# ucuapps/OpenGlue

Measured on NVIDIA H100. Metric: image-pairs/sec at N=M=2048, d=256, 9 GNN layers, 100 Sinkhorn iters, higher is better.
Workload: dtype fp16x3 (fp16 hi/lo operands with power-of-two tensor scales, 3 products, fp32 accumulate)

## Files before the change

openglue_b200/csrc/api.cu:

```cuda
#include "common.cuh"
#include "linear_simt.cuh"
#include "linear_sm90.cuh"
#include "attention_simt.cuh"
#include "attention_sm90.cuh"
#include "sinkhorn.cuh"
#include "sinkhorn_bwd.cuh"
#include "match.cuh"
#include "gt_matches.cuh"
#include "criterion.cuh"
#include "metric_loss.cuh"
#include "collate.cuh"
#include "train_ops.cuh"
#include "superpoint.cuh"
#include "sift.cuh"
#include "kornia_sift.cuh"
#include "features.cuh"
#include "homography.cuh"
#include "optim.cuh"
#include <math.h>
#include <string.h>
#include <vector>

namespace og {

// ... 10 lines not shown
  float* o = out + (int64_t)r * (2 + S);
  if (len) {
    if (!padded_row_real(r, cap, len)) {
      for (int s = 0; s < 2 + S; ++s) o[s] = 0.f;
      return;
    }
    const int b = r / cap;
    wm1 = __ldg(wh + 4 * b) - 1.f;
    hm1 = __ldg(wh + 4 * b + 1) - 1.f;
  }
  o[0] = __fdiv_rn(2.f * __ldg(kpts + 2 * (int64_t)r), wm1) - 1.f;
  o[1] = __fdiv_rn(2.f * __ldg(kpts + 2 * (int64_t)r + 1), hm1) - 1.f;
  for (int s = 0; s < S; ++s) o[2 + s] = __ldg(side + (int64_t)r * S + s);
}

__global__ void __launch_bounds__(256) mask_padded_rows_kernel(const float* __restrict__ src, int64_t rows, int cap, int d,
                                                                const int* __restrict__ len, float* __restrict__ dst) {
  for (int64_t i = blockIdx.x * (int64_t)blockDim.x + threadIdx.x; i < rows * d; i += (int64_t)gridDim.x * blockDim.x)
    dst[i] = padded_row_real(i / d, cap, len) ? __ldg(src + i) : 0.f;
}

__global__ void __launch_bounds__(256) zero_padded_cols_kernel(float* __restrict__ ctx, int B, int d, int cap, const int* __restrict__ len) {
  for (int64_t i = blockIdx.x * (int64_t)blockDim.x + threadIdx.x; i < (int64_t)B * d * cap; i += (int64_t)gridDim.x * blockDim.x) {
    const int b = (int)(i / ((int64_t)d * cap));
    if ((int)(i % cap) >= padded_length(len, b, cap)) ctx[i] = 0.f;
  }
}

__global__ void sinkhorn_consts_kernel(SinkArgs a, float* out) {
  const int b = blockIdx.x * blockDim.x + threadIdx.x;
  if (b >= a.B) return;
  const SinkPair p(a, b);
  out[3 * b] = p.norm; out[3 * b + 1] = p.log_a_last; out[3 * b + 2] = p.log_b_last;
}

struct Layout {
  std::vector<int64_t> kenc_w, kenc_b;
  std::vector<int64_t> qkv_w, qkv_b, fc1_w, fc1_b, fc2_w, fc2_b;
  int64_t proj_w, proj_b, proj_rmix, dustbin, total;
  std::vector<int> kenc_sizes;
};

static int check_config(const og_config* c) {
  OG_CHECK_ARG(c != nullptr, "config is null");
  OG_CHECK_ARG(c->descriptor_dim > 0 && c->num_heads > 0 && c->descriptor_dim % c->num_heads == 0,
               "descriptor_dim %d must be a positive multiple of num_heads %d", c->descriptor_dim, c->num_heads);
  OG_CHECK_ARG(c->num_layers >= 0 && c->num_layers % 2 == 0, "num_layers must be 2 * num_stages");
  OG_CHECK_ARG(c->side_info_size >= 0, "side_info_size < 0");
  OG_CHECK_ARG(c->num_hidden >= 0 && c->num_hidden <= OG_MAX_HIDDEN, "num_hidden out of range");
  OG_CHECK_ARG(c->sinkhorn_iters >= 0 && c->sinkhorn_reg > 0.f, "bad sinkhorn parameters");
  OG_CHECK_ARG(c->descriptor_dim % 4 == 0, "descriptor_dim must be a multiple of 4");
  return OG_OK;
}

static Layout make_layout(const og_config* c) {
  Layout L;
  const int64_t d = c->descriptor_dim;
  L.kenc_sizes.push_back(2 + c->side_info_size);
  for (int i = 0; i < c->num_hidden; ++i) L.kenc_sizes.push_back(c->hidden[i]);
  L.kenc_sizes.push_back((int)d);
  int64_t off = 0;
  auto take = [&](int64_t nfl) { int64_t o = off; off += (nfl + 3) / 4 * 4; return o; };
  for (size_t i = 1; i < L.kenc_sizes.size(); ++i) {
    L.kenc_w.push_back(take((int64_t)L.kenc_sizes[i] * L.kenc_sizes[i - 1]));
    L.kenc_b.push_back(take(L.kenc_sizes[i]));
  }
  for (int l = 0; l < c->num_layers; ++l) {
    L.qkv_w.push_back(take(3 * d * d)); L.qkv_b.push_back(take(3 * d));
    L.fc1_w.push_back(take(4 * d * d)); L.fc1_b.push_back(take(2 * d));
    L.fc2_w.push_back(take(2 * d * d)); L.fc2_b.push_back(take(d));
  }
  L.proj_w = take(d * d); L.proj_b = take(d); L.proj_rmix = take(d); L.dustbin = take(1);
  L.total = off;
  return L;
}

struct Workspace {
  float *in0, *h0, *h1, *x, *qkv, *o, *hid, *g, *ghi, *glo, *sbuf;
  float *q, *khi, *klo, *vthi, *vtlo;
  int64_t ldn, ldm;
  void *sink, *match;
  float* slots;
  int nslots;
  float* desc;
  int64_t lds, sink_bytes, match_bytes, total;
};

static int plan_workspace(const og_config* c, int B, int n, int m, void* base, Workspace* w, bool padded = false) {
  const int64_t d = c->descriptor_dim, R = (int64_t)B * (n + m);
  int maxh = (int)d;
  for (int i = 0; i < c->num_hidden; ++i) maxh = std::max(maxh, c->hidden[i]);
  char* p = static_cast<char*>(base);
  int64_t off = 0;
  auto take = [&](int64_t bytes) { int64_t o = off; off += align_up(bytes, 256); return p ? (void*)(p + o) : nullptr; };
  w->in0 = (float*)take(R * (2 + c->side_info_size) * 4);
  w->h0 = (float*)take(R * maxh * 4);
  w->h1 = (float*)take(R * maxh * 4);
  w->x = (float*)take(R * d * 4);
  w->qkv = (float*)take(R * 3 * d * 4);
  w->o = (float*)take(R * d * 4);
  w->hid = (float*)take(R * 2 * d * 4);
  w->g = (float*)take(R * d * 4);
  w->ghi = (float*)take((int64_t)B * m * d * 4);
  w->glo = (float*)take((int64_t)B * m * d * 4);
  w->ldn = align_up(n, 8); w->ldm = align_up(m, 8);
  w->nslots = 16 * c->num_layers + 16;
  w->slots = (float*)take((int64_t)w->nslots * 4);
  if (c->precision == OG_PREC_TF32X3 || c->precision == OG_PREC_FP16X3) {
    w->q = (float*)take(R * d * 4);
    w->khi = (float*)take(R * d * 4);
    w->klo = (float*)take(R * d * 4);
    w->vthi = (float*)take((int64_t)B * d * (w->ldn + w->ldm) * 4);
    w->vtlo = (float*)take((int64_t)B * d * (w->ldn + w->ldm) * 4);
  } else {
    w->q = w->khi = w->klo = w->vthi = w->vtlo = nullptr;
  }
  w->lds = align_up(m, 4);
  w->sbuf = (float*)take((int64_t)B * n * w->lds * 4);
  w->sink_bytes = sinkhorn_workspace_bytes(B, n, m);
  if (w->sink_bytes < 0) return OG_EUNSUPPORTED;
  w->sink = take(w->sink_bytes);
  w->match_bytes = match_workspace_bytes(B, n, m);
  w->match = take(w->match_bytes);
  w->desc = padded ? (float*)take(R * d * 4) : nullptr;
  w->total = off;
  return OG_OK;
}

static og_linear_args lin(const float* A, int64_t lda, int k, const float* W, const float* bias, int rows, int nout,
                          float* Y, int64_t ldy) {
  og_linear_args a;
  memset(&a, 0, sizeof(a));
  a.A = A; a.lda = lda; a.k1 = k; a.W = W; a.ldw = k; a.bias = bias; a.rows = rows; a.nout = nout; a.batch = 1;
  a.alpha = 1.f; a.Y = Y; a.ldy = ldy;
  return a;
}

template <class T> static T gemm_args(const og_linear_args& a) {
  T t;
  memset(&t, 0, sizeof(t));
  t.A = a.A; t.lda = a.lda; t.strideA = a.strideA; t.A2 = a.A2; t.lda2 = a.lda2; t.strideA2 = a.strideA2;
  t.k1 = a.k1; t.k2 = a.k2;
  t.b_rows_per_batch = a.strideW ? (int)(a.strideW / a.ldw) : 0;
  t.bias = a.bias; t.rows = a.rows; t.nout = a.nout; t.batch = a.batch; t.alpha = a.alpha; t.relu = a.relu;
  t.R = a.R; t.ldr = a.ldr; t.strideR = a.strideR;
  if constexpr (std::is_same<T, TcLinearArgs>::value) {
    t.Y = a.Y; t.ldy = a.ldy; t.strideY = a.strideY; t.Yt = a.Yt; t.ldyt = a.ldyt; t.strideYt = a.strideYt; t.rscale = a.rscale;
  } else {
    t.out[F16_Y] = {a.Y, nullptr, nullptr, a.ldy, a.strideY, nullptr}; t.kind0 = F16_Y; t.nkinds = 1; t.kind_cols = a.nout;
  }
  return t;
}

template <class T, class BT>
static bool gemm_tileable(const og_linear_args& a, const T& t, const BT* Bhi, const BT* Blo) {
  return (!a.strideW || a.strideW % a.ldw == 0) && linear_sm90_eligible(t, Bhi, Blo, a.ldw);
}

template <class T, class BT>
static int gemm_launch(const og_linear_args& a, const T& t, const BT* Bhi, const BT* Blo, cudaStream_t s) {
  const int64_t brows = a.strideW ? (int64_t)t.b_rows_per_batch * (a.batch - 1) + a.nout : a.nout;
  return linear_sm90_launch(t, Bhi, Blo, a.ldw, brows, s);
}

template <class T, class BT>
static int linear_sm90_run(const og_linear_args& a, const T& t, const BT* Bhi, const BT* Blo, const char* who, const char* why,
                           cudaStream_t s) {
  if (!gemm_tileable(a, t, Bhi, Blo))
    return fail(OG_EUNSUPPORTED, "%s: %s", who, a.strideW && a.strideW % a.ldw != 0 ? "strideW must be a multiple of ldw" : why);
  return gemm_launch(a, t, Bhi, Blo, s);
}

struct SplitOut { float *Yhi = nullptr, *Ylo = nullptr, *Ythi = nullptr, *Ytlo = nullptr; };

static TcLinearArgs tc_args(const og_linear_args& a, const SplitOut& so) {
  TcLinearArgs t = gemm_args<TcLinearArgs>(a);
  t.Yhi = so.Yhi; t.Ylo = so.Ylo; t.Ythi = so.Ythi; t.Ytlo = so.Ytlo;
  return t;
}

static int linear_dispatch(const og_linear_args& a, int precision, cudaStream_t s, const float* Whi = nullptr,
                           const float* Wlo = nullptr, const SplitOut& so = SplitOut()) {
  if (precision == OG_PREC_TF32X3 && Whi && Wlo) {
    const TcLinearArgs t = tc_args(a, so);
    if (gemm_tileable(a, t, Whi, Wlo)) return gemm_launch(a, t, Whi, Wlo, s);
  }
  if (so.Yhi || so.Ythi) return fail(OG_EUNSUPPORTED, "split outputs need the tensor-core path");
// ... 935 lines not shown
                   overflow);
}
int og_mask_empty_pairs(const int* len0, const int* len1, int B, int n, int m, int64_t* matches0, float* mscores0, int64_t* matches1,
                        float* mscores1, void* stream) {
  OG_CHECK_ARG(len0 && len1 && matches0 && mscores0 && matches1 && mscores1, "mask_empty_pairs: null pointer");
  OG_CHECK_ARG(B > 0 && n > 0 && m > 0, "mask_empty_pairs: bad sizes");
  const int64_t total = (int64_t)B * ((int64_t)n + m);
  return OG_LAUNCH(mask_empty_pairs_kernel, eltwise_grid(total), 256, 0, (cudaStream_t)stream, len0, len1, B, n, m, matches0, mscores0,
                   matches1, mscores1);
}

int og_homography_pairs(const uint8_t* rgb, int B, int H, int W, int offset, const int32_t* warp_offset, float* image0, float* image1,
                        float* H_true, void* stream) {
  OG_CHECK_ARG(rgb && warp_offset && image0 && image1 && H_true, "homography_pairs: null pointer");
  OG_CHECK_ARG(B >= 1 && B <= 65535, "homography_pairs: B = %d must be in [1, 65535]", B);
  OG_CHECK_ARG(offset >= 1 && H > 0 && W > 0 && 2 * (int64_t)offset < (H < W ? H : W),
               "homography_pairs: offset %d must be >= 1 with 2 offset < min(H, W) = min(%d, %d)", offset, H, W);
  OG_CHECK_ARG((int64_t)HG_ROWS * W <= INT32_MAX, "homography_pairs: W = %d too large", W);
  const int h = H - 2 * offset;
  return OG_LAUNCH(homography_pairs_kernel, dim3(cdiv(h, HG_ROWS), B), HG_THREADS, 0, (cudaStream_t)stream, rgb, H, W, offset,
                   hg_block_width(H, W), warp_offset, image0, image1, H_true);
}

int64_t og_optim_state_bytes(void) { return (int64_t)sizeof(og_optim_state); }
int64_t og_optim_workspace_bytes(int nseg) { return nseg > 0 ? optim_workspace_bytes(nseg) : -1; }

static bool unit_beta(double b) { return b >= 0.0 && b < 1.0; }

static int clip_adam_impl(const og_optim_segment* segments, int nseg, int64_t ntiles, double beta1, double beta2, double eps,
                          double max_norm, double lr_gamma, og_optim_state* state, void* workspace, int64_t workspace_bytes,
                          const int* skip, void* stream) {
  OG_CHECK_ARG(segments && state && workspace, "clip_adam_step: null pointer");
  OG_CHECK_ARG(nseg > 0 && ntiles > 0, "clip_adam_step: nseg = %d and ntiles = %lld must be positive", nseg, (long long)ntiles);
  OG_CHECK_ARG(max_norm > 0.0, "clip_adam_step: max_norm = %g must be positive", max_norm);
  OG_CHECK_ARG(unit_beta(beta1) && unit_beta(beta2), "clip_adam_step: betas (%g, %g) must lie in [0, 1)", beta1, beta2);
  OG_CHECK_ARG(eps >= 0.0, "clip_adam_step: eps = %g must be >= 0", eps);
  OG_CHECK_ARG(lr_gamma > 0.0, "clip_adam_step: lr_gamma = %g must be positive", lr_gamma);
  if (workspace_bytes < optim_workspace_bytes(nseg)) return fail(OG_EWORKSPACE, "clip_adam_step: workspace too small");
  const OptHyper h = {beta1, beta2, eps, max_norm, lr_gamma};
  return optim_step_launch(segments, nseg, ntiles, h, state, workspace, skip, (cudaStream_t)stream);
}

int og_clip_adam_step(const og_optim_segment* segments, int nseg, int64_t ntiles, double beta1, double beta2, double eps,
                      double max_norm, double lr_gamma, og_optim_state* state, void* workspace, int64_t workspace_bytes, void* stream) {
  return clip_adam_impl(segments, nseg, ntiles, beta1, beta2, eps, max_norm, lr_gamma, state, workspace, workspace_bytes, nullptr, stream);
}

int og_clip_adam_step_guarded(const og_optim_segment* segments, int nseg, int64_t ntiles, double beta1, double beta2, double eps,
                              double max_norm, double lr_gamma, og_optim_state* state, void* workspace, int64_t workspace_bytes,
                              const int* skip, void* stream) {
  return clip_adam_impl(segments, nseg, ntiles, beta1, beta2, eps, max_norm, lr_gamma, state, workspace, workspace_bytes, skip, stream);
}

int og_adam_schedule(int64_t nsteps, double lr, double lr_gamma, double beta1, double beta2, double* lr_out, float* step_size,
                     float* bc2_sqrt, void* stream) {
  OG_CHECK_ARG(lr_out && step_size && bc2_sqrt, "adam_schedule: null pointer");
  OG_CHECK_ARG(nsteps > 0 && nsteps < (1 << 24), "adam_schedule: nsteps = %lld must lie in [1, 2^24)", (long long)nsteps);
  OG_CHECK_ARG(unit_beta(beta1) && unit_beta(beta2) && lr_gamma > 0.0, "adam_schedule: bad hyper-parameters");
  cudaStream_t st = (cudaStream_t)stream;
  if (const int rc = OG_LAUNCH(adam_lr_chain_kernel, 1, 1, 0, st, nsteps, lr, lr_gamma, lr_out)) return rc;
  return OG_LAUNCH(adam_scalars_kernel, (unsigned)std::min<int64_t>((nsteps + 255) / 256, 4096), 256, 0, st, nsteps, (const double*)lr_out,
                   beta1, beta2, step_size, bc2_sqrt);
}

static int forward_impl(const og_config* cfg, const float* Wp, const float* Whi, const float* Wlo, const __half* W16h,
                        const __half* W16l, const float* meta16, int B, int n, int m,
                         const float* kpts0,
                         const float* kpts1, const float* side0, const float* side1, const float* desc0,
                         const float* desc1, const float* img_wh, float* ctx0, float* ctx1, float* scores,
                         int64_t* matches0, float* mscores0, int64_t* matches1, float* mscores1, void* workspace,
                         int64_t workspace_bytes, void* stream_, const int* lens = nullptr, const float* pair_wh = nullptr) {
  int rc = check_config(cfg);
  if (rc != OG_OK) return rc;
  const bool padded = lens != nullptr;
  OG_CHECK_ARG(Wp && kpts0 && kpts1 && desc0 && desc1 && (padded ? pair_wh != nullptr : img_wh != nullptr) && scores && workspace,
               "forward: null pointer");
  OG_CHECK_ARG(cfg->side_info_size == 0 || (side0 && side1), "forward: side info missing");
  OG_CHECK_ARG(B > 0 && n > 0 && m > 0, "forward: batch, n, m must be positive");
  OG_CHECK_ARG(cfg->precision == OG_PREC_FP32 || (Whi && Wlo), "forward: the tensor-core modes need packed_hi / packed_lo");
  OG_CHECK_ARG(cfg->precision != OG_PREC_FP16X3 || (W16h && W16l && meta16), "forward: OG_PREC_FP16X3 needs the fp16 weight split (og_pack_f16)");
  const bool tcp = (cfg->precision != OG_PREC_FP32) && cfg->descriptor_dim >= 32;
  const bool f16p = tcp && cfg->precision == OG_PREC_FP16X3 && cfg->descriptor_dim % 64 == 0 &&
                    cfg->descriptor_dim / cfg->num_heads == 64;
  auto WH = [&](int64_t off) { return tcp ? Whi + off : nullptr; };
  auto WL = [&](int64_t off) { return tcp ? Wlo + off : nullptr; };
  OG_CHECK_ARG((reinterpret_cast<uintptr_t>(workspace) & 255) == 0, "forward: workspace must be 256-byte aligned");
  cudaStream_t st = (cudaStream_t)stream_;
  const int prec = cfg->precision == OG_PREC_FP16X3 ? OG_PREC_TF32X3 : cfg->precision;
  const Layout L = make_layout(cfg);
  Workspace w;
  rc = plan_workspace(cfg, B, n, m, workspace, &w, padded);
  if (rc != OG_OK) return rc;
  if (workspace_bytes < w.total) return fail(OG_EWORKSPACE, "forward: workspace %lld < %lld bytes",
                                             (long long)workspace_bytes, (long long)w.total);
  launch_counter() = 0;
  const int d = cfg->descriptor_dim, H = cfg->num_heads, dh = d / H, S = cfg->side_info_size;
  const int R0 = B * n, R1 = B * m, R = R0 + R1;
  float* x0 = w.x; float* x1 = w.x + (int64_t)R0 * d;

  const float* dsc0 = desc0;
  const float* dsc1 = desc1;
  const float wm0 = padded ? 0.f : img_wh[0] - 1.f, hm0 = padded ? 0.f : img_wh[1] - 1.f;
  const float wm1 = padded ? 0.f : img_wh[2] - 1.f, hm1 = padded ? 0.f : img_wh[3] - 1.f;
  const int* len0 = padded ? lens : nullptr;
  const int* len1 = padded ? lens + B : nullptr;
  const float* wh0 = padded ? pair_wh : nullptr;
  const float* wh1 = padded ? pair_wh + 2 : nullptr;
  if ((rc = OG_LAUNCH(kenc_input_kernel, cdiv(R0, 256), 256, 0, st, kpts0, side0, R0, S, wm0, hm0, n, len0, wh0, w.in0)) != OG_OK) return rc;
  if ((rc = OG_LAUNCH(kenc_input_kernel, cdiv(R1, 256), 256, 0, st, kpts1, side1, R1, S, wm1, hm1, m, len1, wh1,
                      w.in0 + (int64_t)R0 * (2 + S))) != OG_OK)
    return rc;
  if (padded) {
    float* d1m = w.desc + (int64_t)R0 * d;
    if ((rc = OG_LAUNCH(mask_padded_rows_kernel, eltwise_grid((int64_t)R0 * d), 256, 0, st, desc0, (int64_t)R0, n, d, lens, w.desc)) != OG_OK)
      return rc;
    if ((rc = OG_LAUNCH(mask_padded_rows_kernel, eltwise_grid((int64_t)R1 * d), 256, 0, st, desc1, (int64_t)R1, m, d, lens + B, d1m)) != OG_OK)
      return rc;
    dsc0 = w.desc; dsc1 = d1m;
  }
  {
    const float* cur = w.in0;
    float* bufs[2] = {w.h0, w.h1};
    const int nl = (int)L.kenc_sizes.size() - 1;
    for (int i = 0; i < nl; ++i) {
      const int kin = L.kenc_sizes[i], kout = L.kenc_sizes[i + 1];
      if (i < nl - 1) {
        og_linear_args a = lin(cur, kin, kin, Wp + L.kenc_w[i], Wp + L.kenc_b[i], R, kout, bufs[i & 1], kout);
        a.relu = 1;
        if ((rc = linear_dispatch(a, OG_PREC_FP32, st)) != OG_OK) return rc;
        cur = bufs[i & 1];
      } else {
        og_linear_args a = lin(cur, kin, kin, Wp + L.kenc_w[i], Wp + L.kenc_b[i], R0, kout, x0, d);
        if (!cfg->no_descriptors) { a.R = dsc0; a.ldr = d; }
        if ((rc = linear_dispatch(a, OG_PREC_FP32, st)) != OG_OK) return rc;
        og_linear_args b = lin(cur + (int64_t)R0 * kin, kin, kin, Wp + L.kenc_w[i], Wp + L.kenc_b[i], R1, kout, x1, d);
        if (!cfg->no_descriptors) { b.R = dsc1; b.ldr = d; }
        if ((rc = linear_dispatch(b, OG_PREC_FP32, st)) != OG_OK) return rc;
      }
    }
  }

  enum class Att { FP32, TF32, F16 };
  const Att att = f16p ? Att::F16 : (tcp && (dh == 32 || dh == 64)) ? Att::TF32 : Att::FP32;
  struct Seqs { int row0, len, count, img; int rows() const { return len * count; } };
  const Seqs img[2] = {{0, n, B, 0}, {R0, m, B, 1}};
  const Seqs all{0, R, 1, 2};
  const bool project_all_rows = att == Att::FP32, mlp_per_image = att == Att::F16;
  auto vt_ld = [&](const Seqs& kv) { return kv.row0 == 0 ? w.ldn : w.ldm; };
  auto vt_off = [&](const Seqs& kv) { return kv.row0 == 0 ? 0 : (int64_t)B * d * w.ldn; };

  int nslot = 0;
  auto new_slot = [&]() -> float* { return w.slots + (nslot < w.nslots - 1 ? nslot++ : w.nslots - 1); };
  float* sx[2] = {};
  struct SeqSlots { float *q, *k, *v, *o; } ss[2] = {};
  auto xslot = [&](const Seqs& g, int i) { return g.img == 2 ? sx[i] : i == 0 ? sx[g.img] : nullptr; };
  __half* kh16 = reinterpret_cast<__half*>(w.khi); __half* kl16 = reinterpret_cast<__half*>(w.klo);
  __half* vth16 = reinterpret_cast<__half*>(w.vthi); __half* vtl16 = reinterpret_cast<__half*>(w.vtlo);
  if (att == Att::F16) {
    OG_CUDA(cudaMemsetAsync(w.slots, 0, (size_t)w.nslots * 4, st));
    sx[0] = sx[1] = new_slot();
    const int64_t nx = (int64_t)R * d;
    if ((rc = OG_LAUNCH(amax_kernel, (unsigned)std::min<int64_t>((nx + 2047) / 2048, 1184), 256, 0, st, w.x, nx, sx[0])) != OG_OK) return rc;
  }
  auto args16 = [&](const og_linear_args& a, float* am0, float* am1, float* am2, int l, int t) {
    F16LinearArgs g = gemm_args<F16LinearArgs>(a);
    g.amax_in[0] = am0; g.amax_in[1] = am1; g.amax_in[2] = am2; g.w_meta = meta16 + ((int64_t)l * 5 + t) * 4;
// ... 50 lines not shown
    if (fuse_qkv && self) return run(q, F16_Y, 3);
    if (fuse_qkv) return (r = run(q, F16_Y, 1)) != OG_OK ? r : run(kv, F16_K, 2);
    for (int k = F16_Y; k < F16_KINDS; ++k)
      if ((r = run(k == F16_Y ? q : kv, k, 1)) != OG_OK) return r;
    return OG_OK;
  };

  auto attend = [&](const Seqs& q, const Seqs& kv) -> int {
    const float scale = (float)pow((double)dh, -0.5);
    const int* klen = padded ? lens + (kv.img == 1 ? B : 0) : nullptr;
    if (att == Att::FP32) {
      const float* qkv_q = w.qkv + (int64_t)q.row0 * 3 * d;
      const float* qkv_kv = w.qkv + (int64_t)kv.row0 * 3 * d;
      AttnArgs a{qkv_q, 3 * d, (int64_t)q.len * 3 * d, qkv_kv + d, 3 * d, (int64_t)kv.len * 3 * d, qkv_kv + 2 * d, 3 * d,
                 (int64_t)kv.len * 3 * d, w.o + (int64_t)q.row0 * d, d, (int64_t)q.len * d, q.count, q.len, kv.len, H, scale, klen};
      return attention_simt_launch(a, dh, st);
    }
    const int64_t ldv = vt_ld(kv), voff = vt_off(kv), k0 = (int64_t)kv.row0 * d;
    TcAttnArgs a{w.q + (int64_t)q.row0 * d, d, (int64_t)q.len * d, w.o + (int64_t)q.row0 * d, d, (int64_t)q.len * d,
                 q.count, q.len, kv.len, H, d, scale, klen};
    if (att == Att::TF32) return attention_tc_launch(a, w.khi + k0, w.klo + k0, d, w.vthi + voff, w.vtlo + voff, ldv, dh, st);
    const SeqSlots& s = ss[q.img == 1];
    return attention_f16_launch(a, F16AttnScales{s.q, s.k, s.v, s.o, 0}, kh16 + k0, kl16 + k0, d, vth16 + voff, vtl16 + voff, ldv, dh, st);
  };

  auto mlp = [&](int l, const Seqs& g) -> int {
    float* xr = w.x + (int64_t)g.row0 * d;
    float* hr = w.hid + (int64_t)g.row0 * 2 * d;
    og_linear_args a1 = lin(xr, d, d, Wp + L.fc1_w[l], Wp + L.fc1_b[l], g.rows(), 2 * d, hr, 2 * d);
    a1.A2 = w.o + (int64_t)g.row0 * d; a1.lda2 = d; a1.k2 = d; a1.ldw = 2 * d; a1.relu = 1;
    og_linear_args a2 = lin(hr, 2 * d, 2 * d, Wp + L.fc2_w[l], Wp + L.fc2_b[l], g.rows(), d, xr, d);
    a2.R = xr; a2.ldr = d;
    int r;
    if (att != Att::F16) {
      if ((r = linear_dispatch(a1, prec, st, WH(L.fc1_w[l]), WL(L.fc1_w[l]))) != OG_OK) return r;
      return linear_dispatch(a2, prec, st, WH(L.fc2_w[l]), WL(L.fc2_w[l]));
    }
    float* sh = new_slot();
    float* sn = new_slot();
    F16LinearArgs g1 = args16(a1, xslot(g, 0), xslot(g, 1), ss[g.img == 1].o, l, 3);
    g1.amax_out = sh;
    if ((r = run16(a1, g1, L.fc1_w[l])) != OG_OK) return r;
    F16LinearArgs g2 = args16(a2, sh, nullptr, nullptr, l, 4);
    g2.amax_out = sn;
    if ((r = run16(a2, g2, L.fc2_w[l])) != OG_OK) return r;
    if (g.img != 1) sx[0] = sn;
    if (g.img != 0) sx[1] = sn;
    return OG_OK;
  };

  for (int l = 0; l < cfg->num_layers; ++l) {
    if (l % 2 == 1) {
      for (int i = 0; i < 2; ++i) {
        if ((rc = project(l, img[i], img[1 - i])) != OG_OK) return rc;
        if ((rc = attend(img[i], img[1 - i])) != OG_OK) return rc;
        if ((rc = mlp(l, img[i])) != OG_OK) return rc;
      }
    } else if (n == m) {
      const Seqs both{0, n, 2 * B, 2};
      if ((rc = project(l, both, both)) != OG_OK) return rc;
      if ((rc = attend(both, both)) != OG_OK) return rc;
      if ((rc = mlp(l, both)) != OG_OK) return rc;
    } else {
      if (project_all_rows && (rc = project(l, all, all)) != OG_OK) return rc;
      for (int i = 0; i < 2; ++i) {
        if (!project_all_rows && (rc = project(l, img[i], img[i])) != OG_OK) return rc;
        if ((rc = attend(img[i], img[i])) != OG_OK) return rc;
      }
      for (int i = 0; i < (mlp_per_image ? 2 : 1); ++i)
        if ((rc = mlp(l, mlp_per_image ? img[i] : all)) != OG_OK) return rc;
    }
  }

  for (int img = 0; img < 2; ++img) {
    const int nn = img ? m : n;
    float* xr = img ? x1 : x0;
    float* gr = w.g + (img ? (int64_t)R0 * d : 0);
    og_linear_args a = lin(xr, d, d, Wp + L.proj_w, Wp + L.proj_b, nn, d, gr, d);
    a.batch = B; a.strideA = (int64_t)nn * d; a.strideY = (int64_t)nn * d;
    a.R = img ? dsc1 : dsc0; a.ldr = d; a.strideR = (int64_t)nn * d; a.rscale = Wp + L.proj_rmix;
    float* ctx = img ? ctx1 : ctx0;
    if (ctx) { a.Yt = ctx; a.ldyt = nn; a.strideYt = (int64_t)d * nn; }
    SplitOut so;
    if (tcp && img == 1) { so.Yhi = w.ghi; so.Ylo = w.glo; }
    if ((rc = linear_dispatch(a, prec, st, WH(L.proj_w), WL(L.proj_w), so)) != OG_OK) return rc;
    if (padded && ctx &&
        (rc = OG_LAUNCH(zero_padded_cols_kernel, eltwise_grid((int64_t)B * d * nn), 256, 0, st, ctx, B, d, nn, lens + (img ? B : 0))) != OG_OK)
      return rc;
  }
  {
    og_linear_args a = lin(w.g, d, d, w.g + (int64_t)R0 * d, nullptr, n, m, w.sbuf, w.lds);
    a.batch = B; a.strideA = (int64_t)n * d; a.strideW = (int64_t)m * d; a.strideY = (int64_t)n * w.lds;
    a.alpha = (float)pow((double)d, -0.5);
    if ((rc = linear_dispatch(a, prec, st, tcp ? w.ghi : nullptr, tcp ? w.glo : nullptr)) != OG_OK) return rc;
  }
  rc = sinkhorn_launch(w.sbuf, w.lds, (int64_t)n * w.lds, Wp + L.dustbin, B, n, m, cfg->sinkhorn_iters,
                       cfg->sinkhorn_reg, scores, w.sink, w.sink_bytes, st, nullptr, nullptr, lens);
  if (rc != OG_OK) return rc;
  if (matches0 || mscores0 || matches1 || mscores1) {
    rc = match_launch(scores, B, n, m, cfg->match_threshold, matches0, mscores0, matches1, mscores1, w.match,
                      w.match_bytes, st, lens);
    if (rc != OG_OK) return rc;
  }
  return OG_OK;
}

int og_superglue_forward(const og_config* cfg, const float* Wp, const float* Whi, const float* Wlo, int B, int n, int m,
                         const float* kpts0, const float* kpts1, const float* side0, const float* side1, const float* desc0,
                         const float* desc1, const float* img_wh, float* ctx0, float* ctx1, float* scores,
                         int64_t* matches0, float* mscores0, int64_t* matches1, float* mscores1, void* workspace,
                         int64_t workspace_bytes, void* stream) {
  if (cfg && cfg->precision == OG_PREC_FP16X3) return fail(OG_EINVAL, "forward: OG_PREC_FP16X3 takes og_superglue_forward_f16");
  return forward_impl(cfg, Wp, Whi, Wlo, nullptr, nullptr, nullptr, B, n, m, kpts0, kpts1, side0, side1, desc0, desc1, img_wh, ctx0, ctx1,
                      scores, matches0, mscores0, matches1, mscores1, workspace, workspace_bytes, stream);
}

int og_superglue_forward_f16(const og_config* cfg, const float* Wp, const float* Whi, const float* Wlo, const void* W16h,
                             const void* W16l, const float* meta16, int B, int n, int m,
                             const float* kpts0, const float* kpts1, const float* side0, const float* side1, const float* desc0,
                             const float* desc1, const float* img_wh, float* ctx0, float* ctx1, float* scores,
                             int64_t* matches0, float* mscores0, int64_t* matches1, float* mscores1, void* workspace,
                             int64_t workspace_bytes, void* stream) {
  return forward_impl(cfg, Wp, Whi, Wlo, static_cast<const __half*>(W16h), static_cast<const __half*>(W16l), meta16, B, n, m, kpts0, kpts1,
                      side0, side1, desc0, desc1, img_wh, ctx0, ctx1, scores, matches0, mscores0, matches1, mscores1, workspace,
                      workspace_bytes, stream);
}

int64_t og_workspace_bytes_padded(const og_config* cfg, int batch, int n, int m) {
  if (check_config(cfg) != OG_OK) return -1;
  if (batch <= 0 || n <= 0 || m <= 0) return fail(OG_EINVAL, "batch, n, m must be positive");
  Workspace w;
  if (plan_workspace(cfg, batch, n, m, nullptr, &w, true) != OG_OK) return -1;
  return w.total;
}

int og_superglue_forward_padded(const og_config* cfg, const float* Wp, const float* Whi, const float* Wlo, const void* W16h,
                                const void* W16l, const float* meta16, int B, int n, int m, const int* lengths,
                                const float* image_sizes, const float* kpts0, const float* kpts1, const float* side0,
                                const float* side1, const float* desc0, const float* desc1, float* ctx0, float* ctx1, float* scores,
                                int64_t* matches0, float* mscores0, int64_t* matches1, float* mscores1, void* workspace,
                                int64_t workspace_bytes, void* stream) {
  OG_CHECK_ARG(lengths && image_sizes, "forward_padded: null lengths / image_sizes");
  OG_CHECK_ARG(B <= 65535, "forward_padded: batch %d > 65535", B);
  return forward_impl(cfg, Wp, Whi, Wlo, static_cast<const __half*>(W16h), static_cast<const __half*>(W16l), meta16, B, n, m, kpts0, kpts1,
                      side0, side1, desc0, desc1, nullptr, ctx0, ctx1, scores, matches0, mscores0, matches1, mscores1, workspace,
                      workspace_bytes, stream, lengths, image_sizes);
}

int64_t og_f16_meta_floats(const og_config* cfg) {
  if (check_config(cfg) != OG_OK) return -1;
  return (int64_t)cfg->num_layers * 5 * 4;
}

int og_weight_split_f16(const float* w, const float* bias, int rows, int cols, void* hi16, void* lo16, float* meta, void* stream) {
  OG_CHECK_ARG(w && hi16 && lo16 && meta && rows > 0 && cols > 0, "weight_split_f16: bad arguments");
  cudaStream_t st = (cudaStream_t)stream;
  OG_CUDA(cudaMemsetAsync(meta, 0, 4 * sizeof(float), st));
  int rc;
  if ((rc = OG_LAUNCH(weight_meta_kernel, cdiv(rows, 8), 256, 0, st, w, bias, rows, cols, meta)) != OG_OK) return rc;
  const int64_t nel = (int64_t)rows * cols;
  if ((rc = OG_LAUNCH(split_f16_kernel, (unsigned)((nel + 255) / 256), 256, 0, st, w, static_cast<__half*>(hi16), static_cast<__half*>(lo16),
                      nel, meta)) != OG_OK)
    return rc;
  return OG_LAUNCH(finish_meta_kernel, 1, 1, 0, st, meta);
}

int og_pack_f16(const og_config* cfg, const float* Wp, void* hi16, void* lo16, float* meta, void* stream) {
  int rc = check_config(cfg);
  if (rc != OG_OK) return rc;
  OG_CHECK_ARG(Wp && hi16 && lo16 && meta, "pack_f16: null pointer");
  const Layout L = make_layout(cfg);
  const int64_t d = cfg->descriptor_dim;
  __half* h = static_cast<__half*>(hi16); __half* lo = static_cast<__half*>(lo16);
  for (int l = 0; l < cfg->num_layers; ++l) {
    struct T { int64_t woff, boff; int rows, cols; } ts[5] = {
      {L.qkv_w[l], L.qkv_b[l], (int)d, (int)d}, {L.qkv_w[l] + d * d, L.qkv_b[l] + d, (int)d, (int)d},
      {L.qkv_w[l] + 2 * d * d, L.qkv_b[l] + 2 * d, (int)d, (int)d},
      {L.fc1_w[l], L.fc1_b[l], (int)(2 * d), (int)(2 * d)}, {L.fc2_w[l], L.fc2_b[l], (int)d, (int)(2 * d)}};
    for (int t = 0; t < 5; ++t)
      if ((rc = og_weight_split_f16(Wp + ts[t].woff, Wp + ts[t].boff, ts[t].rows, ts[t].cols, h + ts[t].woff, lo + ts[t].woff,
                                    meta + ((int64_t)l * 5 + t) * 4, stream)) != OG_OK) return rc;
  }
  return OG_OK;
}
// ... 57 lines not shown
```

openglue_b200/csrc/match.cuh:

```cuda
#pragma once
#include "common.cuh"
#include <math_constants.h>

namespace og {

constexpr int MATCH_ROW_CHUNK = 64;

__device__ __forceinline__ int2 match_lengths(const int* lens, int b, int B, int n, int m) {
  if (!lens) return make_int2(n, m);
  return make_int2(padded_length(lens, b, n), padded_length(lens + B, b, m));
}

__global__ void __launch_bounds__(256) match_rowmax_kernel(const float* __restrict__ scores, int n, int m, const int* lens,
                                                            float* __restrict__ rowval, int* __restrict__ rowidx) {
  const int b = blockIdx.y;
  const int row = blockIdx.x * 8 + (threadIdx.x >> 5), lane = threadIdx.x & 31;
  const int2 len = match_lengths(lens, b, gridDim.y, n, m);
  if (row >= len.x) return;
  const float* src = scores + ((int64_t)b * (n + 1) + row) * (m + 1);
  float best = -CUDART_INF_F; int bi = 0x7fffffff;
  for (int c = lane; c < len.y; c += 32) {
    const float x = __ldg(src + c);
    if (x > best || bi == 0x7fffffff) { best = x; bi = c; }
  }
#pragma unroll
  for (int off = 16; off > 0; off >>= 1) {
    const float ov = __shfl_xor_sync(0xffffffffu, best, off);
    const int oi = __shfl_xor_sync(0xffffffffu, bi, off);
    if (ov > best || (ov == best && oi < bi)) { best = ov; bi = oi; }
  }
  if (lane == 0) { rowval[(int64_t)b * n + row] = best; rowidx[(int64_t)b * n + row] = bi; }
}

__global__ void __launch_bounds__(256) match_colmax_kernel(const float* __restrict__ scores, int n, int m, const int* lens, int chunks,
                                                            float* __restrict__ pval, int* __restrict__ pidx) {
  const int b = blockIdx.z, chunk = blockIdx.y;
  const int c = blockIdx.x * blockDim.x + threadIdx.x;
  const int2 len = match_lengths(lens, b, gridDim.z, n, m);
  if (c >= len.y) return;
  const int r0 = chunk * MATCH_ROW_CHUNK, r1 = min(r0 + MATCH_ROW_CHUNK, len.x);
  if (r0 >= r1) {
    pval[((int64_t)b * chunks + chunk) * m + c] = -CUDART_INF_F;
    pidx[((int64_t)b * chunks + chunk) * m + c] = r0;
    return;
  }
  const float* src = scores + (int64_t)b * (n + 1) * (m + 1) + c;
  float best = __ldg(src + (int64_t)r0 * (m + 1)); int bi = r0;
  for (int r = r0 + 1; r < r1; ++r) {
    const float x = __ldg(src + (int64_t)r * (m + 1));
    if (x > best) { best = x; bi = r; }
  }
  pval[((int64_t)b * chunks + chunk) * m + c] = best;
  pidx[((int64_t)b * chunks + chunk) * m + c] = bi;
}

__global__ void __launch_bounds__(256) match_colreduce_kernel(int n, int m, int chunks, const float* __restrict__ pval,
                                                               const int* __restrict__ pidx, int* __restrict__ colidx) {
  const int b = blockIdx.y;
  const int c = blockIdx.x * blockDim.x + threadIdx.x;
  if (c >= m) return;
  float best = pval[((int64_t)b * chunks) * m + c]; int bi = pidx[((int64_t)b * chunks) * m + c];
  for (int k = 1; k < chunks; ++k) {
    const float x = pval[((int64_t)b * chunks + k) * m + c];
    if (x > best) { best = x; bi = pidx[((int64_t)b * chunks + k) * m + c]; }
  }
  colidx[(int64_t)b * m + c] = bi;
}

__global__ void __launch_bounds__(256) match_finalize_kernel(int n, int m, const int* lens, float thr, const float* __restrict__ rowval,
                                                              const int* __restrict__ rowidx, const int* __restrict__ colidx,
                                                              int64_t* __restrict__ matches0, float* __restrict__ mscores0,
                                                              int64_t* __restrict__ matches1, float* __restrict__ mscores1) {
  const int b = blockIdx.y;
  const int t = blockIdx.x * blockDim.x + threadIdx.x;
  const int* ri = rowidx + (int64_t)b * n;
  const int* ci = colidx + (int64_t)b * m;
  const float* rv = rowval + (int64_t)b * n;
  const int2 len = match_lengths(lens, b, gridDim.y, n, m);
  if (t >= len.x && t < n) {
    if (matches0) matches0[(int64_t)b * n + t] = -1;
    if (mscores0) mscores0[(int64_t)b * n + t] = 0.f;
  }
  if (t >= len.y && t < m) {
    if (matches1) matches1[(int64_t)b * m + t] = -1;
    if (mscores1) mscores1[(int64_t)b * m + t] = 0.f;
  }
  if (t < len.x) {
    const int j = ri[t];
    const bool mutual = (ci[j] == t);
    const float ms = mutual ? expf(rv[t]) : 0.f;
    const bool valid = mutual && (ms > thr);
    if (matches0) matches0[(int64_t)b * n + t] = valid ? (int64_t)j : -1;
    if (mscores0) mscores0[(int64_t)b * n + t] = ms;
  }
  if (t < len.y && (matches1 || mscores1)) {
    const int i = ci[t];
    const bool mutual1 = (ri[i] == t);
    const bool mutual0_i = (ci[ri[i]] == i);
    const float ms0_i = mutual0_i ? expf(rv[i]) : 0.f;
    const float ms1 = mutual1 ? ms0_i : 0.f;
    const bool valid1 = mutual1 && (mutual0_i && ms0_i > thr);
    if (matches1) matches1[(int64_t)b * m + t] = valid1 ? (int64_t)i : -1;
    if (mscores1) mscores1[(int64_t)b * m + t] = ms1;
  }
}

inline int64_t match_workspace_bytes(int B, int n, int m) {
  const int chunks = cdiv(n, MATCH_ROW_CHUNK);
  return align_up((int64_t)B * n * 4, 256) * 2 + align_up((int64_t)B * m * 4, 256) +
         align_up((int64_t)B * chunks * m * 4, 256) * 2;
}

inline int match_launch(const float* scores, int B, int n, int m, float thr, int64_t* matches0, float* mscores0, int64_t* matches1,
                        float* mscores1, void* ws, int64_t ws_bytes, cudaStream_t stream, const int* lens = nullptr) {
  if (ws_bytes < match_workspace_bytes(B, n, m)) return fail(OG_EWORKSPACE, "match: workspace too small");
  const int chunks = cdiv(n, MATCH_ROW_CHUNK);
  char* w = static_cast<char*>(ws);
  float* rowval = reinterpret_cast<float*>(w); w += align_up((int64_t)B * n * 4, 256);
  int* rowidx = reinterpret_cast<int*>(w); w += align_up((int64_t)B * n * 4, 256);
  int* colidx = reinterpret_cast<int*>(w); w += align_up((int64_t)B * m * 4, 256);
  float* pval = reinterpret_cast<float*>(w); w += align_up((int64_t)B * chunks * m * 4, 256);
  int* pidx = reinterpret_cast<int*>(w);
  int rc;
  if ((rc = OG_LAUNCH(match_rowmax_kernel, dim3(cdiv(n, 8), B), 256, 0, stream, scores, n, m, lens, rowval, rowidx))) return rc;
  if ((rc = OG_LAUNCH(match_colmax_kernel, dim3(cdiv(m, 256), chunks, B), 256, 0, stream, scores, n, m, lens, chunks, pval, pidx)))
    return rc;
  if ((rc = OG_LAUNCH(match_colreduce_kernel, dim3(cdiv(m, 256), B), 256, 0, stream, n, m, chunks, pval, pidx, colidx))) return rc;
  return OG_LAUNCH(match_finalize_kernel, dim3(cdiv(std::max(n, m), 256), B), 256, 0, stream, n, m, lens, thr, rowval, rowidx,
                   colidx, matches0, mscores0, matches1, mscores1);
}

}
```

Before: 504.5.

## Run score GEMM in fp16x3 and fuse row/column argmax into one pass

For fp16x3 mode the descriptor score GEMM now runs on the fp16 sm90 GEMM. The second image's projected descriptors are split into fp16 hi/lo with amax-derived scales, instead of the tf32 hi/lo split. The match step also drops the separate row-max kernel: the column-max kernel now computes per-column-block row partial argmaxes via warp shuffles and shared memory, and finalize reduces those partials. This saves a full read of the score matrix and moves the score GEMM to cheaper fp16 tensor-core math, at the cost of extra amax/split launches and slightly different tie-breaking.

```diff
diff --git a/openglue_b200/csrc/api.cu b/openglue_b200/csrc/api.cu
--- a/openglue_b200/csrc/api.cu
+++ b/openglue_b200/csrc/api.cu
@@ -116,6 +116,7 @@
   void *sink, *match;
   float* slots;
   int nslots;
+  float* gmeta;
   float* desc;
   int64_t lds, sink_bytes, match_bytes, total;
 };
@@ -137,6 +138,7 @@
   w->g = (float*)take(R * d * 4);
   w->ghi = (float*)take((int64_t)B * m * d * 4);
   w->glo = (float*)take((int64_t)B * m * d * 4);
+  w->gmeta = (float*)take(8 * 4);
   w->ldn = align_up(n, 8); w->ldm = align_up(m, 8);
   w->nslots = 16 * c->num_layers + 16;
   w->slots = (float*)take((int64_t)w->nslots * 4);
@@ -1238,6 +1240,7 @@
   const bool tcp = (cfg->precision != OG_PREC_FP32) && cfg->descriptor_dim >= 32;
   const bool f16p = tcp && cfg->precision == OG_PREC_FP16X3 && cfg->descriptor_dim % 64 == 0 &&
                     cfg->descriptor_dim / cfg->num_heads == 64;
+  const bool f16_scores = tcp && cfg->precision == OG_PREC_FP16X3 && cfg->descriptor_dim % 64 == 0;
   auto WH = [&](int64_t off) { return tcp ? Whi + off : nullptr; };
   auto WL = [&](int64_t off) { return tcp ? Wlo + off : nullptr; };
   OG_CHECK_ARG((reinterpret_cast<uintptr_t>(workspace) & 255) == 0, "forward: workspace must be 256-byte aligned");
@@ -1454,7 +1457,7 @@
     float* ctx = img ? ctx1 : ctx0;
     if (ctx) { a.Yt = ctx; a.ldyt = nn; a.strideYt = (int64_t)d * nn; }
     SplitOut so;
-    if (tcp && img == 1) { so.Yhi = w.ghi; so.Ylo = w.glo; }
+    if (tcp && !f16_scores && img == 1) { so.Yhi = w.ghi; so.Ylo = w.glo; }
     if ((rc = linear_dispatch(a, prec, st, WH(L.proj_w), WL(L.proj_w), so)) != OG_OK) return rc;
     if (padded && ctx &&
         (rc = OG_LAUNCH(zero_padded_cols_kernel, eltwise_grid((int64_t)B * d * nn), 256, 0, st, ctx, B, d, nn, lens + (img ? B : 0))) != OG_OK)
@@ -1464,14 +1467,28 @@
     og_linear_args a = lin(w.g, d, d, w.g + (int64_t)R0 * d, nullptr, n, m, w.sbuf, w.lds);
     a.batch = B; a.strideA = (int64_t)n * d; a.strideW = (int64_t)m * d; a.strideY = (int64_t)n * w.lds;
     a.alpha = (float)pow((double)d, -0.5);
-    if ((rc = linear_dispatch(a, prec, st, tcp ? w.ghi : nullptr, tcp ? w.glo : nullptr)) != OG_OK) return rc;
+    if (f16_scores) {
+      __half* g1h = reinterpret_cast<__half*>(w.ghi); __half* g1l = reinterpret_cast<__half*>(w.glo);
+      float* am0 = w.gmeta + 4;
+      const int64_t n0 = (int64_t)R0 * d, n1 = (int64_t)R1 * d;
+      OG_CUDA(cudaMemsetAsync(w.gmeta, 0, 8 * sizeof(float), st));
+      if ((rc = OG_LAUNCH(amax_kernel, (unsigned)std::min<int64_t>((n1 + 2047) / 2048, 1184), 256, 0, st, a.W, n1, w.gmeta)) != OG_OK) return rc;
+      if ((rc = OG_LAUNCH(split_f16_kernel, (unsigned)((n1 + 255) / 256), 256, 0, st, a.W, g1h, g1l, n1, w.gmeta)) != OG_OK) return rc;
+      if ((rc = OG_LAUNCH(finish_meta_kernel, 1, 1, 0, st, w.gmeta)) != OG_OK) return rc;
+      if ((rc = OG_LAUNCH(amax_kernel, (unsigned)std::min<int64_t>((n0 + 2047) / 2048, 1184), 256, 0, st, w.g, n0, am0)) != OG_OK) return rc;
+      F16LinearArgs g = gemm_args<F16LinearArgs>(a);
+      g.amax_in[0] = am0; g.w_meta = w.gmeta;
+      if ((rc = linear_sm90_run(a, g, g1h, g1l, "forward", "the score GEMM is not tileable by the fp16 GEMM", st)) != OG_OK) return rc;
+    } else if ((rc = linear_dispatch(a, prec, st, tcp ? w.ghi : nullptr, tcp ? w.glo : nullptr)) != OG_OK) {
+      return rc;
+    }
   }
   rc = sinkhorn_launch(w.sbuf, w.lds, (int64_t)n * w.lds, Wp + L.dustbin, B, n, m, cfg->sinkhorn_iters,
                        cfg->sinkhorn_reg, scores, w.sink, w.sink_bytes, st, nullptr, nullptr, lens);
   if (rc != OG_OK) return rc;
   if (matches0 || mscores0 || matches1 || mscores1) {
     rc = match_launch(scores, B, n, m, cfg->match_threshold, matches0, mscores0, matches1, mscores1, w.match,
-                      w.match_bytes, st, lens);
+                      w.match_bytes, st, lens, true);
     if (rc != OG_OK) return rc;
   }
   return OG_OK;
diff --git a/openglue_b200/csrc/match.cuh b/openglue_b200/csrc/match.cuh
--- a/openglue_b200/csrc/match.cuh
+++ b/openglue_b200/csrc/match.cuh
@@ -32,26 +32,62 @@
   if (lane == 0) { rowval[(int64_t)b * n + row] = best; rowidx[(int64_t)b * n + row] = bi; }
 }
 
+constexpr int MATCH_COLS_PER_THREAD = 4, MATCH_COL_BLOCK = 256 * MATCH_COLS_PER_THREAD;
+__device__ __forceinline__ bool match_better(float v, int i, float best, int bi) { return v > best || (v == best && i < bi); }
+
 __global__ void __launch_bounds__(256) match_colmax_kernel(const float* __restrict__ scores, int n, int m, const int* lens, int chunks,
-                                                            float* __restrict__ pval, int* __restrict__ pidx) {
-  const int b = blockIdx.z, chunk = blockIdx.y;
-  const int c = blockIdx.x * blockDim.x + threadIdx.x;
+                                                            float* __restrict__ pval, int* __restrict__ pidx, float* __restrict__ rval,
+                                                            int* __restrict__ ridx) {
+  __shared__ float sv[8][MATCH_ROW_CHUNK];
+  __shared__ int si[8][MATCH_ROW_CHUNK];
+  const int b = blockIdx.z, chunk = blockIdx.y, warp = threadIdx.x >> 5, lane = threadIdx.x & 31;
+  const int cb = blockIdx.x * MATCH_COL_BLOCK + threadIdx.x;
   const int2 len = match_lengths(lens, b, gridDim.z, n, m);
-  if (c >= len.y) return;
   const int r0 = chunk * MATCH_ROW_CHUNK, r1 = min(r0 + MATCH_ROW_CHUNK, len.x);
-  if (r0 >= r1) {
-    pval[((int64_t)b * chunks + chunk) * m + c] = -CUDART_INF_F;
-    pidx[((int64_t)b * chunks + chunk) * m + c] = r0;
-    return;
+  const float* src = scores + (int64_t)b * (n + 1) * (m + 1);
+  float best[MATCH_COLS_PER_THREAD]; int bi[MATCH_COLS_PER_THREAD];
+#pragma unroll
+  for (int k = 0; k < MATCH_COLS_PER_THREAD; ++k) { best[k] = -CUDART_INF_F; bi[k] = r0; }
+  for (int r = r0; r < r1; ++r) {
+    const float* row = src + (int64_t)r * (m + 1);
+    float rb = -CUDART_INF_F; int rj = 0x7fffffff;
+#pragma unroll
+    for (int k = 0; k < MATCH_COLS_PER_THREAD; ++k) {
+      const int c = cb + 256 * k;
+      if (c < len.y) {
+        const float x = __ldg(row + c);
+        if (r == r0 || x > best[k]) { best[k] = x; bi[k] = r; }
+        if (x > rb || rj == 0x7fffffff) { rb = x; rj = c; }
+      }
+    }
+    if (rval) {
+#pragma unroll
+      for (int off = 16; off > 0; off >>= 1) {
+        const float ov = __shfl_xor_sync(0xffffffffu, rb, off);
+        const int oi = __shfl_xor_sync(0xffffffffu, rj, off);
+        if (match_better(ov, oi, rb, rj)) { rb = ov; rj = oi; }
+      }
+      if (lane == 0) { sv[warp][r - r0] = rb; si[warp][r - r0] = rj; }
+    }
   }
-  const float* src = scores + (int64_t)b * (n + 1) * (m + 1) + c;
-  float best = __ldg(src + (int64_t)r0 * (m + 1)); int bi = r0;
-  for (int r = r0 + 1; r < r1; ++r) {
-    const float x = __ldg(src + (int64_t)r * (m + 1));
-    if (x > best) { best = x; bi = r; }
+#pragma unroll
+  for (int k = 0; k < MATCH_COLS_PER_THREAD; ++k) {
+    const int c = cb + 256 * k;
+    if (c < len.y) {
+      pval[((int64_t)b * chunks + chunk) * m + c] = best[k];
+      pidx[((int64_t)b * chunks + chunk) * m + c] = bi[k];
+    }
   }
-  pval[((int64_t)b * chunks + chunk) * m + c] = best;
-  pidx[((int64_t)b * chunks + chunk) * m + c] = bi;
+  if (rval) {
+    __syncthreads();
+    for (int i = threadIdx.x; i < r1 - r0; i += blockDim.x) {
+      float v = sv[0][i]; int j = si[0][i];
+      for (int w = 1; w < 8; ++w)
+        if (match_better(sv[w][i], si[w][i], v, j)) { v = sv[w][i]; j = si[w][i]; }
+      rval[((int64_t)b * n + r0 + i) * gridDim.x + blockIdx.x] = v;
+      ridx[((int64_t)b * n + r0 + i) * gridDim.x + blockIdx.x] = j;
+    }
+  }
 }
 
 __global__ void __launch_bounds__(256) match_colreduce_kernel(int n, int m, int chunks, const float* __restrict__ pval,
@@ -67,15 +103,21 @@
   colidx[(int64_t)b * m + c] = bi;
 }
 
-__global__ void __launch_bounds__(256) match_finalize_kernel(int n, int m, const int* lens, float thr, const float* __restrict__ rowval,
-                                                              const int* __restrict__ rowidx, const int* __restrict__ colidx,
+__global__ void __launch_bounds__(256) match_finalize_kernel(int n, int m, const int* lens, float thr, int rparts,
+                                                              const float* __restrict__ rowval, const int* __restrict__ rowidx,
+                                                              const int* __restrict__ colidx,
                                                               int64_t* __restrict__ matches0, float* __restrict__ mscores0,
                                                               int64_t* __restrict__ matches1, float* __restrict__ mscores1) {
   const int b = blockIdx.y;
   const int t = blockIdx.x * blockDim.x + threadIdx.x;
-  const int* ri = rowidx + (int64_t)b * n;
   const int* ci = colidx + (int64_t)b * m;
-  const float* rv = rowval + (int64_t)b * n;
+  auto row = [&](int i, float& v) {
+    const int64_t p = ((int64_t)b * n + i) * rparts;
+    v = rowval[p]; int j = rowidx[p];
+    for (int k = 1; k < rparts; ++k)
+      if (match_better(rowval[p + k], rowidx[p + k], v, j)) { v = rowval[p + k]; j = rowidx[p + k]; }
+    return j;
+  };
   const int2 len = match_lengths(lens, b, gridDim.y, n, m);
   if (t >= len.x && t < n) {
     if (matches0) matches0[(int64_t)b * n + t] = -1;
@@ -86,18 +128,21 @@
     if (mscores1) mscores1[(int64_t)b * m + t] = 0.f;
   }
   if (t < len.x) {
-    const int j = ri[t];
+    float rv;
+    const int j = row(t, rv);
     const bool mutual = (ci[j] == t);
-    const float ms = mutual ? expf(rv[t]) : 0.f;
+    const float ms = mutual ? expf(rv) : 0.f;
     const bool valid = mutual && (ms > thr);
     if (matches0) matches0[(int64_t)b * n + t] = valid ? (int64_t)j : -1;
     if (mscores0) mscores0[(int64_t)b * n + t] = ms;
   }
   if (t < len.y && (matches1 || mscores1)) {
     const int i = ci[t];
-    const bool mutual1 = (ri[i] == t);
-    const bool mutual0_i = (ci[ri[i]] == i);
-    const float ms0_i = mutual0_i ? expf(rv[i]) : 0.f;
+    float rv;
+    const int ri = row(i, rv);
+    const bool mutual1 = (ri == t);
+    const bool mutual0_i = (ci[ri] == i);
+    const float ms0_i = mutual0_i ? expf(rv) : 0.f;
     const float ms1 = mutual1 ? ms0_i : 0.f;
     const bool valid1 = mutual1 && (mutual0_i && ms0_i > thr);
     if (matches1) matches1[(int64_t)b * m + t] = valid1 ? (int64_t)i : -1;
@@ -106,27 +151,29 @@
 }
 
 inline int64_t match_workspace_bytes(int B, int n, int m) {
-  const int chunks = cdiv(n, MATCH_ROW_CHUNK);
-  return align_up((int64_t)B * n * 4, 256) * 2 + align_up((int64_t)B * m * 4, 256) +
+  const int chunks = cdiv(n, MATCH_ROW_CHUNK), rparts = cdiv(m, MATCH_COL_BLOCK);
+  return align_up((int64_t)B * n * rparts * 4, 256) * 2 + align_up((int64_t)B * m * 4, 256) +
          align_up((int64_t)B * chunks * m * 4, 256) * 2;
 }
 
 inline int match_launch(const float* scores, int B, int n, int m, float thr, int64_t* matches0, float* mscores0, int64_t* matches1,
-                        float* mscores1, void* ws, int64_t ws_bytes, cudaStream_t stream, const int* lens = nullptr) {
+                        float* mscores1, void* ws, int64_t ws_bytes, cudaStream_t stream, const int* lens = nullptr,
+                        bool one_pass = false) {
   if (ws_bytes < match_workspace_bytes(B, n, m)) return fail(OG_EWORKSPACE, "match: workspace too small");
-  const int chunks = cdiv(n, MATCH_ROW_CHUNK);
+  const int chunks = cdiv(n, MATCH_ROW_CHUNK), cblocks = cdiv(m, MATCH_COL_BLOCK), rparts = one_pass ? cblocks : 1;
   char* w = static_cast<char*>(ws);
-  float* rowval = reinterpret_cast<float*>(w); w += align_up((int64_t)B * n * 4, 256);
-  int* rowidx = reinterpret_cast<int*>(w); w += align_up((int64_t)B * n * 4, 256);
+  float* rowval = reinterpret_cast<float*>(w); w += align_up((int64_t)B * n * cblocks * 4, 256);
+  int* rowidx = reinterpret_cast<int*>(w); w += align_up((int64_t)B * n * cblocks * 4, 256);
   int* colidx = reinterpret_cast<int*>(w); w += align_up((int64_t)B * m * 4, 256);
   float* pval = reinterpret_cast<float*>(w); w += align_up((int64_t)B * chunks * m * 4, 256);
   int* pidx = reinterpret_cast<int*>(w);
   int rc;
-  if ((rc = OG_LAUNCH(match_rowmax_kernel, dim3(cdiv(n, 8), B), 256, 0, stream, scores, n, m, lens, rowval, rowidx))) return rc;
-  if ((rc = OG_LAUNCH(match_colmax_kernel, dim3(cdiv(m, 256), chunks, B), 256, 0, stream, scores, n, m, lens, chunks, pval, pidx)))
+  if (!one_pass && (rc = OG_LAUNCH(match_rowmax_kernel, dim3(cdiv(n, 8), B), 256, 0, stream, scores, n, m, lens, rowval, rowidx))) return rc;
+  if ((rc = OG_LAUNCH(match_colmax_kernel, dim3(cblocks, chunks, B), 256, 0, stream, scores, n, m, lens, chunks, pval, pidx,
+                      one_pass ? rowval : nullptr, one_pass ? rowidx : nullptr)))
     return rc;
   if ((rc = OG_LAUNCH(match_colreduce_kernel, dim3(cdiv(m, 256), B), 256, 0, stream, n, m, chunks, pval, pidx, colidx))) return rc;
-  return OG_LAUNCH(match_finalize_kernel, dim3(cdiv(std::max(n, m), 256), B), 256, 0, stream, n, m, lens, thr, rowval, rowidx,
+  return OG_LAUNCH(match_finalize_kernel, dim3(cdiv(std::max(n, m), 256), B), 256, 0, stream, n, m, lens, thr, rparts, rowval, rowidx,
                    colidx, matches0, mscores0, matches1, mscores1);
 }
 
```

New measurement: 511.9, median of 6. 1.01x the previous value.
